# uguryagmur/RealTimeObjectDetection

Measured on AMD Instinct MI355X. Metric: frames/sec YOLOv3 608x608 bs=8 (Darknet.forward + write_results; 2 batches in flight, write_results_async on a second stream), higher is better.
Workload: dtype f16x2-split (3 MFMA products, f32 accumulate); 1 GPU; YOLOv3 cfg 608x608 batch=8 per GPU, split-f16 MFMA conv + fused head + GPU NMS (BASELINE configs[2]); precision=f16s3, tiles=autotune (this run), parallelism=frame-shard x1, in_flight_batches=2, detections_last_step=1699, candidates_last_step=1914, f16_range_overflow=False

## Files before the change

### include/rtod.h

```cpp
#ifndef RTOD_H
#define RTOD_H

#include <stddef.h>
#include <stdint.h>

#ifdef __cplusplus
extern "C" {
#endif

typedef enum rtod_status {
    RTOD_OK = 0,
    RTOD_E_ARG = -1,
    RTOD_E_HIP = -2,
    RTOD_E_CFG = -3,
    RTOD_E_STATE = -4,
    RTOD_E_SIZE = -5
} rtod_status;

typedef struct rtod_plan rtod_plan;

typedef struct rtod_plan_info {
    int32_t n_layers;
    int32_t n_launches;
    int32_t height, width, max_batch;
// ... 14 lines not shown
    int32_t fused_pointwise;
    int64_t flops_per_frame;
    int64_t bytes_per_frame;
    int64_t weight_bytes;
} rtod_launch_info;

int rtod_version(void);
int rtod_last_error(char* buf, size_t len);
int rtod_device_count(int* out);

int rtod_plan_create(const char* cfg_text, size_t len, int height, int width, int max_batch,
                     int device, rtod_plan** out);
int rtod_plan_create_rect(const char* cfg_text, size_t len, int height, int width, int max_batch,
                          int device, rtod_plan** out);
int rtod_plan_destroy(rtod_plan* plan);
int rtod_plan_get_info(const rtod_plan* plan, rtod_plan_info* out);
int rtod_plan_get_launch(const rtod_plan* plan, int index, rtod_launch_info* out);
int rtod_plan_describe(const rtod_plan* plan, char* buf, size_t len, size_t* needed);
int rtod_plan_pack_weights(const rtod_plan* plan, const float* w, size_t n_floats, float* out, size_t capacity_floats,
                           size_t* needed_floats);
const char* rtod_conv_variant_name(int variant);
int rtod_conv_kernel_name(int variant, int epilogue, char* buf, size_t len);
int rtod_plan_launch_kernel_name(const rtod_plan* plan, int index, char* buf, size_t len);
int rtod_plan_set_precision(rtod_plan* plan, int mode);
int rtod_plan_set_option(rtod_plan* plan, const char* name, int value);
int rtod_plan_set_overflow_flag(rtod_plan* plan, int32_t* flag_dev);

int rtod_plan_load_weights(rtod_plan* plan, const float* w, size_t n_floats);

int rtod_forward(rtod_plan* plan, const float* x_dev, int batch, float* out_dev, void* stream);
int rtod_plan_autotune(rtod_plan* plan, const float* x_dev, int batch, float* out_dev, void* stream);
int rtod_plan_get_tiles(const rtod_plan* plan, int batch, int* variants, int capacity);
int rtod_plan_set_tiles(rtod_plan* plan, int batch, const int* variants, int count);
int rtod_forward_timed(rtod_plan* plan, const float* x_dev, int batch, float* out_dev,
                       void* stream, float* launch_ms);
int rtod_plan_set_train_decode(rtod_plan* plan, int train);
int rtod_plan_finish_decode(rtod_plan* plan, float* pred_dev, int batch, void* stream);
int rtod_plan_set_keep_all_layers(rtod_plan* plan, int keep);
int rtod_plan_layer_shape(const rtod_plan* plan, int layer, int* c, int* h, int* w);
int rtod_plan_read_layer(rtod_plan* plan, int layer, int batch, float* out_dev_nchw, void* stream);
int rtod_plan_bn_batch_stats(rtod_plan* plan, int layer, double* mean_host, double* var_host, int channels, void* stream);
int rtod_plan_bn_update_running(rtod_plan* plan, int batch, float* const* running_mean_dev, float* const* running_var_dev, int n_bn,
                                double momentum, void* stream);

int rtod_predict_transform(const float* raw_dev, int batch, int attrs, int grid, int n_anchors,
                           const float* anchors_wh, int inp_dim, int train, float* out_dev,
// ... 46 lines not shown
```

### realtimeobjectdetection_amd/_ffi.py

```python
import ctypes as C
import os

_HERE = os.path.dirname(os.path.abspath(__file__))
LIB_PATH = os.path.join(_HERE, os.environ.get("RTOD_LIB", "librtod.so"))


class RtodError(RuntimeError):
    def __init__(self, code, msg):
        super().__init__(f"librtod error {code}: {msg}")
        self.code = code


class PlanInfo(C.Structure):
    _fields_ = [("n_layers", C.c_int32), ("n_launches", C.c_int32), ("height", C.c_int32),
                ("width", C.c_int32), ("max_batch", C.c_int32), ("total_rows", C.c_int32),
                ("attrs", C.c_int32), ("n_weight_floats", C.c_int64),
                ("conv_flops_per_frame", C.c_int64), ("arena_bytes", C.c_int64),
                ("packed_weight_bytes", C.c_int64)]


class LaunchInfo(C.Structure):
    _fields_ = [("layer", C.c_int32), ("kind", C.c_int32), ("variant", C.c_int32),
                ("ksize", C.c_int32), ("stride", C.c_int32), ("cin", C.c_int32), ("cout", C.c_int32),
                ("hout", C.c_int32), ("wout", C.c_int32), ("fused_residual", C.c_int32),
                ("fused_decode", C.c_int32), ("fused_pointwise", C.c_int32), ("flops_per_frame", C.c_int64),
                ("bytes_per_frame", C.c_int64), ("weight_bytes", C.c_int64)]


class YoloHead(C.Structure):
    _fields_ = [("grid_h", C.c_int), ("grid_w", C.c_int), ("stride", C.c_int), ("n_anchors", C.c_int), ("anchors", C.c_int * 16)]


SIGNATURES = {
    "rtod_version": (C.c_int, []),
    "rtod_last_error": (C.c_int, [C.c_char_p, C.c_size_t]),
    "rtod_device_count": (C.c_int, [C.POINTER(C.c_int)]),
    "rtod_plan_create": (C.c_int, [C.c_char_p, C.c_size_t, C.c_int, C.c_int, C.c_int, C.c_int, C.POINTER(C.c_void_p)]),
    "rtod_plan_create_rect": (C.c_int, [C.c_char_p, C.c_size_t, C.c_int, C.c_int, C.c_int, C.c_int, C.POINTER(C.c_void_p)]),
    "rtod_plan_destroy": (C.c_int, [C.c_void_p]),
    "rtod_plan_get_info": (C.c_int, [C.c_void_p, C.POINTER(PlanInfo)]),
    "rtod_plan_get_launch": (C.c_int, [C.c_void_p, C.c_int, C.POINTER(LaunchInfo)]),
    "rtod_plan_describe": (C.c_int, [C.c_void_p, C.c_char_p, C.c_size_t, C.POINTER(C.c_size_t)]),
    "rtod_plan_pack_weights": (C.c_int, [C.c_void_p, C.c_void_p, C.c_size_t, C.c_void_p, C.c_size_t, C.POINTER(C.c_size_t)]),
    "rtod_conv_variant_name": (C.c_char_p, [C.c_int]),
    "rtod_conv_kernel_name": (C.c_int, [C.c_int, C.c_int, C.c_char_p, C.c_size_t]),
    "rtod_plan_launch_kernel_name": (C.c_int, [C.c_void_p, C.c_int, C.c_char_p, C.c_size_t]),
    "rtod_plan_set_precision": (C.c_int, [C.c_void_p, C.c_int]),
    "rtod_plan_set_option": (C.c_int, [C.c_void_p, C.c_char_p, C.c_int]),
    "rtod_plan_set_overflow_flag": (C.c_int, [C.c_void_p, C.c_void_p]),
    "rtod_plan_autotune": (C.c_int, [C.c_void_p, C.c_void_p, C.c_int, C.c_void_p, C.c_void_p]),
    "rtod_plan_get_tiles": (C.c_int, [C.c_void_p, C.c_int, C.POINTER(C.c_int), C.c_int]),
    "rtod_plan_set_tiles": (C.c_int, [C.c_void_p, C.c_int, C.POINTER(C.c_int), C.c_int]),
    "rtod_plan_load_weights": (C.c_int, [C.c_void_p, C.c_void_p, C.c_size_t]),
    "rtod_forward": (C.c_int, [C.c_void_p, C.c_void_p, C.c_int, C.c_void_p, C.c_void_p]),
    "rtod_forward_timed": (C.c_int, [C.c_void_p, C.c_void_p, C.c_int, C.c_void_p, C.c_void_p, C.POINTER(C.c_float)]),
    "rtod_plan_set_train_decode": (C.c_int, [C.c_void_p, C.c_int]),
    "rtod_plan_finish_decode": (C.c_int, [C.c_void_p, C.c_void_p, C.c_int, C.c_void_p]),
    "rtod_plan_set_keep_all_layers": (C.c_int, [C.c_void_p, C.c_int]),
    "rtod_plan_layer_shape": (C.c_int, [C.c_void_p, C.c_int, C.POINTER(C.c_int), C.POINTER(C.c_int), C.POINTER(C.c_int)]),
    "rtod_plan_read_layer": (C.c_int, [C.c_void_p, C.c_int, C.c_int, C.c_void_p, C.c_void_p]),
    "rtod_plan_bn_batch_stats": (C.c_int, [C.c_void_p, C.c_int, C.c_void_p, C.c_void_p, C.c_int, C.c_void_p]),
    "rtod_plan_bn_update_running": (C.c_int, [C.c_void_p, C.c_int, C.c_void_p, C.c_void_p, C.c_int, C.c_double, C.c_void_p]),
    "rtod_predict_transform": (C.c_int, [C.c_void_p, C.c_int, C.c_int, C.c_int, C.c_int, C.POINTER(C.c_float), C.c_int, C.c_int, C.c_void_p, C.c_void_p]),
    "rtod_confidence_mask": (C.c_int, [C.c_void_p, C.c_int64, C.c_int, C.c_float, C.c_void_p, C.c_void_p]),
    "rtod_bbox_iou": (C.c_int, [C.c_void_p, C.c_void_p, C.c_int, C.c_int, C.c_void_p, C.c_void_p]),
    "rtod_prep_image": (C.c_int, [C.c_void_p, C.c_int, C.c_int, C.c_int, C.c_int, C.c_void_p, C.c_void_p]),
    "rtod_prep_frames": (C.c_int, [C.c_void_p, C.c_int, C.c_int, C.c_int, C.c_int, C.c_int, C.c_int, C.c_void_p, C.c_void_p]),
    "rtod_write_results_workspace": (C.c_int, [C.c_int, C.c_int, C.POINTER(C.c_size_t)]),
# ... 44 lines not shown
```

### realtimeobjectdetection_amd/csrc/capi.cpp

```cpp
#include <cstring>
#include <new>

#include "plan.h"

namespace rtod { const std::string& last_error_string(); }
using namespace rtod;

struct rtod_plan { Plan p; };

#define RTOD_GUARD_BEGIN try {
#define RTOD_GUARD_END                                                                   \
    } catch (const std::bad_alloc&) { set_error("out of host memory"); return RTOD_E_ARG; } \
      catch (const std::exception& e) { set_error("internal error: %s", e.what()); return RTOD_E_ARG; } \
      catch (...) { set_error("internal error"); return RTOD_E_ARG; }

extern "C" {

int rtod_version(void) { return 100; }

int rtod_last_error(char* buf, size_t len) {
    if (!buf || !len) return RTOD_E_ARG;
    const std::string& e = last_error_string();
    const size_t n = e.size() < len - 1 ? e.size() : len - 1;
    memcpy(buf, e.data(), n);
    buf[n] = 0;
    return RTOD_OK;
// ... 85 lines not shown
    if (int rc = plan->p.pack_weights(w, n_floats, packed)) return rc;
    if (!packed.empty()) memcpy(out, packed.data(), sizeof(float) * packed.size());
    return RTOD_OK;
    RTOD_GUARD_END
}

const char* rtod_conv_variant_name(int variant) {
    if (variant == 100 + STEM2_VARIANT) return "conv_stem2_f16s3<2 x 4x16, stem + 3x3 s2 + 1x1>";
    if (variant >= 100) { const TileRef t = family_of(variant - 100); return t ? t.fam->info(t.mode).name : ""; }
    if (variant < 0 || variant % 10 >= CV_COUNT || variant / 10 > 2) return "";
    static const char* const kSliced[2][CV_COUNT] = {
        {"conv_igemm_f32<128x128,w64x64,k-slices>", "conv_igemm_f32<128x64,w64x32,k-slices>", "conv_igemm_f32<64x64,w32x32,k-slices>", "conv_igemm_f32<128x32,w32x32,k-slices>"},
        {"conv_igemm_f32<128x128,w64x64,wg per k-slice>", "conv_igemm_f32<128x64,w64x32,wg per k-slice>", "conv_igemm_f32<64x64,w32x32,wg per k-slice>", "conv_igemm_f32<128x32,w32x32,wg per k-slice>"}};
    if (variant >= 10) return kSliced[variant / 10 - 1][variant % 10];
    return conv_variant_info(variant).name;
}

int rtod_conv_kernel_name(int variant, int epilogue, char* buf, size_t len) {
    if (!buf || len == 0) { set_error("conv_kernel_name: null buffer"); return RTOD_E_ARG; }
    int n = -1;
    if (variant >= 100) { const TileRef t = family_of(variant - 100); if (t) n = t.fam->kernel_name(t.mode, epilogue, buf, len); }
    else n = conv_f32_kernel_name(variant, buf, len);
    if (n < 0 || (size_t)n >= len) { set_error("conv_kernel_name: unknown variant %d or buffer too small", variant); return RTOD_E_ARG; }
    return RTOD_OK;
}

int rtod_plan_launch_kernel_name(const rtod_plan* plan, int index, char* buf, size_t len) {
    RTOD_GUARD_BEGIN
    if (!plan || !buf || len == 0 || index < 0 || index >= (int)plan->p.launches.size()) { set_error("launch_kernel_name: bad args"); return RTOD_E_ARG; }
    rtod_launch_info li;
    plan->p.fill_launch_info(index, &li, plan->p.tuned.empty() ? plan->p.max_batch : plan->p.tuned.rbegin()->first);
    buf[0] = 0;
    if (li.kind != LK_CONV || li.flops_per_frame == 0) return RTOD_OK;
    int epi = li.fused_decode ? 2 : (li.fused_pointwise ? (li.fused_residual ? 4 : 3) : (li.fused_residual ? 1 : 0));
    if (plan->p.precision == 2 && li.variant >= 100) epi |= EPI_F16;
    if (plan->p.raw_launch(plan->p.launches[index]) && li.variant >= 100) epi = EPI_RAW;
    int n = -1;
    if (li.variant == 100 + STEM2_VARIANT) n = conv_stem2_kernel_name(li.fused_pointwise, buf, len);
    else return rtod_conv_kernel_name(li.variant, epi, buf, len);
    if (n < 0 || (size_t)n >= len) { set_error("launch_kernel_name: buffer too small"); return RTOD_E_ARG; }
    return RTOD_OK;
    RTOD_GUARD_END
}

int rtod_plan_set_precision(rtod_plan* plan, int mode) {
    if (!plan || mode < 0 || mode > 2) { set_error("set_precision: mode must be 0 (fp32), 1 (f16 split) or 2 (plain f16)"); return RTOD_E_ARG; }
// ... 258 lines not shown
```

### realtimeobjectdetection_amd/csrc/plan.h

```cpp
#pragma once
#include <functional>
#include <map>
#include <string>
#include <vector>

#include "rtod_internal.h"

namespace rtod {

enum LayerType { LT_CONV = 0, LT_SHORTCUT, LT_ROUTE, LT_UPSAMPLE, LT_MAXPOOL, LT_YOLO };
const char* layer_type_name(int t);

struct Layer {
    int index = 0;
    int type = LT_CONV;
    int cin = 0, cout = 0, hin = 0, win = 0, hout = 0, wout = 0;
    int size = 0, stride = 1, pad = 0;
    bool bn = false;
    int act = 0;
    bool nearest = false;
    bool decode_v5 = false;
    int pool_pad = 0;
    std::vector<int> srcs;
    std::vector<std::pair<int, int>> anchors;
// ... 61 lines not shown
    double* d_bn_partial = nullptr;
    int64_t bn_partial_count = 0;
    float* d_bn_raw = nullptr;
    int64_t bn_raw_floats = 0;
    float* d_scratch = nullptr;
    int64_t scratch_floats = 0;
    bool weights_loaded = false;
    int train_decode = 0;
    int precision = 0;
    bool keep_all = false;
    bool opt_fuse_pointwise = true;
    bool opt_stem_kernel = true;
    bool opt_band_kernel = true;
    bool opt_bn_batch_stats = false;
    bool opt_bn_batch_split = false;
    bool opt_bn_split_narrow = false;
    bool opt_fuse_bn_pool = true;
    bool opt_k_slices = true;
    bool opt_k_slice_workgroups = true;
    bool opt_k_slices_split = false;
    bool opt_stem2_kernel = true;
    bool opt_patch_kernel = true;
    bool opt_ring_kernel = true;
    bool opt_pwd_kernel = true;
    bool opt_fuse_shortcut = true;
    bool opt_fuse_decode = true;
    bool opt_zero_copy_concat = true;
    bool opt_narrow_cin = false;
    bool opt_stem_pool = false;
    bool opt_fuse_stem_pool = true;
    int opt_force_f16s3_variant = -1;
    int opt_force_f32_variant = -1;
    int32_t* overflow_flag = nullptr;
    std::vector<hipEvent_t> events;

    ~Plan();
    int parse(const std::string& cfg_text);
    int resolve_shapes();
    int plan_buffers();
    DecodeArgs decode_args(const Layer& yolo) const;
    int replan_or(const std::function<void()>& restore);
    void assign_arena();
    void layout_weights();
    bool uses_split(const Layer& L) const;
    int check_split_supported(int mode) const;
    int pack_weights(const float* w, size_t n, std::vector<float>& packed) const;
// ... 45 lines not shown
```

### realtimeobjectdetection_amd/csrc/plan_build.cpp

```cpp
#include "plan.h"

#include <algorithm>
#include <cstdarg>
#include <sstream>

namespace rtod {

static thread_local std::string g_err;

void set_error(const char* fmt, ...) {
    char buf[1024];
    va_list ap;
    va_start(ap, fmt);
    vsnprintf(buf, sizeof(buf), fmt, ap);
    va_end(ap);
    g_err = buf;
}
const std::string& last_error_string() { return g_err; }

int hip_fail(hipError_t e, const char* what) {
    if (e == hipSuccess) return RTOD_OK;
    set_error("HIP error %d (%s) at %s", (int)e, hipGetErrorString(e), what);
    return RTOD_E_HIP;
}
// ... 14 lines not shown
}

static int resolve_alias(const std::vector<Layer>& layers, int i) {
    while (layers[i].alias_of >= 0) i = layers[i].alias_of;
    return i;
}

void Plan::reset_planning() {
    for (auto& L : layers) { L.fused_into = -1; L.fused_away = false; L.buf = -1; L.coff = 0; L.alias_of = -1; L.bn_pool = -1; }
    bufs.clear(); launches.clear(); convs.clear(); input_buf = -1;
    tuned.clear(); tune_cache.clear(); tuning.clear();
}

int Plan::set_option(const char* name, int value) {
    if (!name) { set_error("set_option: null name"); return RTOD_E_ARG; }
    if (d_weights) { set_error("set_option: must be called before rtod_plan_load_weights"); return RTOD_E_STATE; }
    static const struct { const char* name; bool Plan::*flag; } kFlags[] = {
        {"fuse_pointwise", &Plan::opt_fuse_pointwise}, {"ring_kernel", &Plan::opt_ring_kernel}, {"pwd_kernel", &Plan::opt_pwd_kernel},
        {"stem2_kernel", &Plan::opt_stem2_kernel}, {"k_slices", &Plan::opt_k_slices}, {"bn_batch_stats", &Plan::opt_bn_batch_stats},
        {"bn_batch_split", &Plan::opt_bn_batch_split}, {"bn_split_narrow", &Plan::opt_bn_split_narrow}, {"fuse_bn_pool", &Plan::opt_fuse_bn_pool},
        {"k_slice_workgroups", &Plan::opt_k_slice_workgroups}, {"k_slices_split", &Plan::opt_k_slices_split}, {"patch_kernel", &Plan::opt_patch_kernel},
        {"stem_kernel", &Plan::opt_stem_kernel}, {"band_kernel", &Plan::opt_band_kernel}, {"fuse_shortcut", &Plan::opt_fuse_shortcut},
        {"fuse_decode", &Plan::opt_fuse_decode}, {"zero_copy_concat", &Plan::opt_zero_copy_concat}, {"narrow_cin", &Plan::opt_narrow_cin},
        {"stem_pool", &Plan::opt_stem_pool}, {"fuse_stem_pool", &Plan::opt_fuse_stem_pool},
    };
    const std::string k(name);
    bool* flag = nullptr; int* num = nullptr;
    for (const auto& f : kFlags) if (k == f.name) flag = &(this->*f.flag);
    if (k == "force_f16s3_variant") num = &opt_force_f16s3_variant;
    else if (k == "force_f32_variant") num = &opt_force_f32_variant;
    else if (!flag) { set_error("set_option: unknown option '%s'", name); return RTOD_E_ARG; }
    if (flag == &opt_bn_batch_stats && value && height != width) { set_error("set_option: bn_batch_stats is not supported on a rectangular plan (%dx%d)", height, width); return RTOD_E_ARG; }
    const bool old_flag = flag ? *flag : false; const int old_num = num ? *num : 0;
    if (flag) *flag = value != 0; else *num = value;
    return replan_or([&] { if (flag) *flag = old_flag; else *num = old_num; });
}

int Plan::replan_or(const std::function<void()>& restore) {
    reset_planning();
    int rc = plan_buffers();
    if (!rc && precision >= 1) rc = check_split_supported(precision);
    if (rc) {
        const std::string msg = last_error_string();
        restore();
        reset_planning();
        (void)plan_buffers();
        set_error("%s", msg.c_str());
// ... 371 lines not shown
```

### realtimeobjectdetection_amd/csrc/plan_tiles.cpp

```cpp
#include "plan.h"

#include <algorithm>
#include <mutex>

namespace rtod {

int Plan::choose_variant(const Layer& L, int batch) const {
    if (opt_force_f32_variant >= 0 && opt_force_f32_variant < CV_COUNT) return opt_force_f32_variant;
    if (L.cout <= 32) return CV_128x32;
    if (L.cout <= 64) return CV_128x64;
    const int64_t M = (int64_t)batch * L.hout * L.wout;
    const int64_t big = ((M + 127) / 128) * ((L.cout + 127) / 128);
    return big >= 512 ? CV_128x128 : CV_64x64;
}

int Plan::f32_slice_mode(const Launch& l, int batch, int variant) const {
    const PackedConv& pc = convs[l.conv_slot];
    if (pc.split || pc.stem || pc.slice_chunks <= 0) return 0;
    const Layer& L = layers[l.layer];
    const ConvVariantInfo& vi = conv_variant_info(variant);
    const int64_t M = (int64_t)batch * L.hout * L.wout;
    const int64_t tiles = ((M + vi.bm - 1) / vi.bm) * ((L.cout + vi.bn - 1) / vi.bn);
    const int64_t S = (pc.Kpad / 32 + pc.slice_chunks - 1) / pc.slice_chunks;
    return (opt_k_slice_workgroups && d_scratch && tiles < 512 && S * M * pc.Npad <= scratch_floats) ? 2 : 1;
}

bool Plan::tile_legal(const Launch& l, int v) const {
    const TileRef t = family_of(v);
    if (!t || l.kind != LK_CONV || l.conv_slot < 0 || !convs[l.conv_slot].split) return false;
    const PackedConv& pc = convs[l.conv_slot];
    const Layer& L = layers[l.layer];
    if (precision == 2 && !t.f16()) return false;
    if (raw_launch(l) && !t.raw()) return false;
    if (pc.narrow || t.is(TF_C16)) return pc.narrow && t.is(TF_C16);
    if (pc.ks_chunks > 0 || t.is(TF_KS)) return pc.ks_chunks > 0 && t.is(TF_KS);
    if (pc.band) return t.is(TF_BAND) && conv_band_mode_valid(t.mode, L.cin, L.hin, L.win);
    const bool hosts_pw = l.pw_guest >= 0 && pw_active(), plain = l.out_layer != -2 && !hosts_pw, same_map = L.hout == L.hin && L.wout == L.win;
    switch (t.fam->id) {
        case TF_GENERIC: return !(hosts_pw && t.fam->info(t.mode).bn < L.cout);
        case TF_BAND: return t.bandd_wide() && opt_band_kernel && plain && same_map && pc.Npad % 128 == 0 && pc.K == pc.Kpad &&
                             conv_bandd_wide_supported(L.size, L.stride, L.pad, pc.cin_p, L.win);
        case TF_RING: return !hosts_pw && L.act <= 1;
        case TF_PWD: return opt_pwd_kernel && plain && same_map && conv_pwd_supported(L.size, L.stride, L.pad, pc.cin_p);
        case TF_PATCH: return plain && L.act <= 1 && L.hout == L.hin && conv_patch_supported(L.size, L.stride, L.pad, L.cin, L.cout) &&
                              conv_patch_mode_valid(t.mode, L.cin, L.cout);
    }
    return false;
}

int Plan::default_tile(const Launch& l, int batch) const {
    const PackedConv& pc = convs[l.conv_slot];
    const Layer& L = layers[l.layer];
    const int64_t M = (int64_t)batch * L.hout * L.wout;
    if (pc.narrow) return tile_id(TF_C16, conv_c16_default_mode(L.cout, M));
    if (pc.ks_chunks > 0) return tile_id(TF_KS, ((M + 63) / 64) * ((L.cout + 63) / 64) < 512 ? 1 : 0);
    if (pc.band) {
        if (precision != 2 && !raw_launch(l)) return tile_id(TF_BAND, conv_band_default_mode(L.cin, L.hin, L.win));
        const TileFamily& B = tile_family(TF_BAND);
        for (int m = 0; m < B.modes; ++m) if (tile_legal(l, B.base + m)) return B.base + m;
        return B.base + B.f16_from;
    }
    const int64_t gn = (L.cout + 127) / 128;
    const int g = L.cout <= 64 ? HV_128x64 : ((M + 127) / 128) * gn >= 512 ? HV_128x128 : ((M + 63) / 64) * gn >= 512 ? HV_64x128 : HV_64x64;
    return tile_legal(l, g) ? g : HV_128x128_8W;
}

int Plan::variant_for(const Launch& l, int batch) const {
    int want = opt_force_f16s3_variant;
    if (want < 0) {
        auto it = tuned.find(batch);
        const size_t idx = &l - &launches[0];
        if (it != tuned.end() && idx < it->second.size()) want = it->second[idx];
    }
    int v = want >= 0 && tile_legal(l, want) ? want : default_tile(l, batch);
    if (family_of(v).ks_sched_b() && !(opt_k_slice_workgroups && ks_sched_b_fits(l, batch))) --v;
    return v;
}

std::vector<int> Plan::tile_candidates(const Launch& l, int batch) const {
    static const int kOrder[TF_COUNT] = {TF_GENERIC, TF_PATCH, TF_BAND, TF_PWD, TF_RING, TF_C16, TF_KS};
    const int cout = layers[l.layer].cout;
    const bool ks_b = opt_k_slice_workgroups && ks_sched_b_fits(l, batch);
    std::vector<int> cand;
    for (int f : kOrder) {
        if ((f == TF_RING && !opt_ring_kernel) || (f == TF_PATCH && !opt_patch_kernel)) continue;
        const TileFamily& F = tile_family(f);
        for (int m = 0; m < F.modes; ++m) {
            const int bn = F.info(m).bn;
            const bool too_wide = f == TF_GENERIC || f == TF_RING ? bn > 64 && bn > 2 * ((cout + 63) / 64 * 64)
                                : f == TF_PATCH ? bn > 64 && bn > cout
                                : f == TF_PWD ? bn > 128 && bn > (cout + 127) / 128 * 128 : false;
            if (too_wide || (family_of(F.base + m).ks_sched_b() && !ks_b) || !tile_legal(l, F.base + m)) continue;
            cand.push_back(F.base + m);
        }
    }
    return cand;
}

int Plan::launch_split_variant(ConvArgs& a, const PackedConv& pc, int v, hipStream_t s) const {
    const TileRef t = family_of(v);
    if (!t) { set_error("variant %d is no split-f16 tile", v); return RTOD_E_STATE; }
    if (precision == 2 && !t.f16()) { set_error("variant %d has no plain-f16 instance", v); return RTOD_E_STATE; }
    if (a.raw_out && !t.raw()) { set_error("variant %d has no raw-sum instance", v); return RTOD_E_STATE; }
// ... 7 lines not shown
    }
    if (pc.band != t.is(TF_BAND) && !(t.bandd_wide() && !pc.band)) {
        set_error(pc.band ? "variant %d requested for a band layer" : "band variant %d requested for a layer without band weights", v);
        return RTOD_E_STATE;
    }
    if (t.is(TF_KS)) {
        a.slice_chunks = pc.ks_chunks;
        a.partial = nullptr; a.partial_floats = 0;
        if (t.ks_sched_b()) { a.partial = d_scratch; a.partial_floats = scratch_floats; }
    }
    return t.fam->launch(a, t.mode, s);
}

static std::mutex g_tune_mutex;
static std::map<std::vector<int>, int> g_tune_memo;

int Plan::tune_launch(size_t li, ConvArgs& a, int batch, hipStream_t s) {
    const Launch& l = launches[li];
    const Layer& L = layers[l.layer];
    const bool pw = a.pw_wh != nullptr;
    const std::vector<int> key = {L.cin, L.cout, L.size, L.stride, L.hout, L.wout, l.in2_layer >= 0, l.out_layer == -2, pw ? a.pw_cout : 0,
                                  convs[l.conv_slot].band ? 1 : 0, opt_ring_kernel ? 1 : 0, opt_patch_kernel ? 1 : 0, opt_pwd_kernel ? 1 : 0, L.act,
                                  precision, L.hin, L.win, L.pad, convs[l.conv_slot].ks_chunks, opt_k_slice_workgroups ? 1 : 0,
                                  a.raw_out ? 1 : 0};
    auto it = tune_cache.find(key);
    if (it != tune_cache.end()) { tuning[li] = it->second; return RTOD_OK; }
    std::vector<int> gkey = key; gkey.push_back(device); gkey.push_back(batch);
    {
        std::lock_guard<std::mutex> lock(g_tune_mutex);
        auto git = g_tune_memo.find(gkey);
        if (git != g_tune_memo.end()) { tuning[li] = git->second; tune_cache[key] = git->second; return RTOD_OK; }
    }
    hipEvent_t e0, e1;
    RTOD_HIP(hipEventCreate(&e0)); RTOD_HIP(hipEventCreate(&e1));
    const std::vector<int> cand = tile_candidates(l, batch);
    int best_v = variant_for(l, batch);
    int rc = RTOD_OK;
    auto time_variant = [&](int v, int reps, int per, float& out_ms) -> int {
        out_ms = 1e30f;
        for (int rep = 0; rep < reps; ++rep) {
            (void)hipEventRecord(e0, s);
            for (int r = 0; r < per; ++r) { const int q = launch_split_variant(a, convs[l.conv_slot], v, s); if (q) return q; }
            (void)hipEventRecord(e1, s);
            if (hipEventSynchronize(e1) != hipSuccess) return hip_fail(hipGetLastError(), "autotune sync");
            float ms = 0.f; (void)hipEventElapsedTime(&ms, e0, e1);
            out_ms = std::min(out_ms, ms / per);
        }
// ... 57 lines not shown
```

### realtimeobjectdetection_amd/csrc/rtod_internal.h

```cpp
#pragma once
#include <hip/hip_runtime.h>
#if defined(RTOD_STAMPS) && !defined(RTOD_DIAG)
#define RTOD_DIAG 1
#endif
#include <algorithm>
#include <atomic>
#include <cstdint>
#include <cstdio>
#include <string>
#include <vector>

#include "../../include/rtod.h"

namespace rtod {

void set_error(const char* fmt, ...);
int hip_fail(hipError_t e, const char* what);

#define RTOD_HIP(expr)                                              \
    do {                                                            \
        hipError_t _e = (expr);                                     \
        if (_e != hipSuccess) return ::rtod::hip_fail(_e, #expr);   \
    } while (0)

// ... 159 lines not shown
constexpr int PATCH_VARIANT_BASE = 110;
bool conv_patch_supported(int ksize, int stride, int pad, int cin, int cout);
const ConvVariantInfo& conv_patch_mode_info(int mode);
int conv_patch_kernel_name(int mode, int epi, char* buf, size_t len);
int launch_conv_patch_f16s3(const ConvArgs& a, int mode, hipStream_t s);

constexpr int C16_MODES = 4;
constexpr int C16_VARIANT_BASE = 140;
constexpr bool conv_c16_supported(int cin) { return cin == 16; }
const ConvVariantInfo& conv_c16_mode_info(int mode);
int conv_c16_default_mode(int cout, int64_t m);
int conv_c16_kernel_name(int mode, int epi, char* buf, size_t len);
int launch_conv_c16_f16s3(const ConvArgs& a, int mode, hipStream_t s);

constexpr int KS_TILES = 3;
constexpr int KS_MODES = 2 * KS_TILES;
constexpr int KS_VARIANT_BASE = 150;
constexpr int64_t KS_SCRATCH_FLOATS = 8ll << 20;
const ConvVariantInfo& conv_ks_mode_info(int mode);
int conv_ks_slices(const ConvArgs& a);
int conv_ks_kernel_name(int mode, int epi, char* buf, size_t len);
int launch_conv_ks_f16s3(const ConvArgs& a, int mode, hipStream_t s);

enum TileFamilyId { TF_GENERIC = 0, TF_BAND, TF_RING, TF_PWD, TF_PATCH, TF_C16, TF_KS, TF_COUNT };
struct TileFamily {
    int id, base, modes;
    int f16_from;
    int raw_from;
    const ConvVariantInfo& (*info)(int mode);
    int (*kernel_name)(int mode, int epi, char* buf, size_t len);
    int (*launch)(const ConvArgs& a, int mode, hipStream_t s);
};
struct TileRef {
    const TileFamily* fam; int mode;
    explicit operator bool() const { return fam != nullptr; }
    bool is(int family) const { return fam && fam->id == family; }
    bool f16() const { return fam && mode >= fam->f16_from; }
    bool raw() const { return fam && mode >= fam->raw_from; }
    bool ks_sched_b() const { return is(TF_KS) && (mode & 1); }
    bool bandd_wide() const { return is(TF_BAND) && mode == BANDD_WIDE_MODE; }
};
TileRef family_of(int v);
const TileFamily& tile_family(int family);
inline int tile_id(int family, int mode) { return tile_family(family).base + mode; }

int launch_conv_stem(const float* x_nchw, const float* w, const float* bias, const View& out, int B, int H, int W,
                     int Ho, int Wo, int stride, int Cout, int leaky, hipStream_t s);
// ... 52 lines not shown
```

### realtimeobjectdetection_amd/csrc/split_tiles.cpp

```cpp
#include "rtod_internal.h"

namespace rtod {

static const TileFamily kFamilies[TF_COUNT] = {
    {TF_GENERIC, 0, HV_COUNT, 0, 0, conv_f16s3_variant_info, conv_f16s3_kernel_name, launch_conv_f16s3},
    {TF_BAND, BAND_VARIANT_BASE, BAND_MODES, BAND_LDS_MODES, BAND_LDS_MODES, conv_band_mode_info, conv_band_kernel_name, launch_conv_band_f16s3},
    {TF_RING, RING_VARIANT_BASE, RING_MODES, RING_MODES, RING_MODES, conv_ring_mode_info, conv_ring_kernel_name, launch_conv_ring_f16s3},
    {TF_PWD, PWD_VARIANT_BASE, PWD_MODES, 0, 0, conv_pwd_mode_info, conv_pwd_kernel_name, launch_conv_pwd_f16s3},
    {TF_PATCH, PATCH_VARIANT_BASE, PATCH_MODES, PATCH_MODES, PATCH_MODES, conv_patch_mode_info, conv_patch_kernel_name, launch_conv_patch_f16s3},
    {TF_C16, C16_VARIANT_BASE, C16_MODES, 0, 0, conv_c16_mode_info, conv_c16_kernel_name, launch_conv_c16_f16s3},
    {TF_KS, KS_VARIANT_BASE, KS_MODES, 0, KS_MODES, conv_ks_mode_info, conv_ks_kernel_name, launch_conv_ks_f16s3},
};
static_assert(HV_COUNT <= BAND_VARIANT_BASE, "generic tile ids end where the band family's begin");
static_assert(BAND_VARIANT_BASE + BAND_MODES <= RING_VARIANT_BASE, "band tile ids end where the ring family's begin");
static_assert(RING_VARIANT_BASE + RING_MODES <= PWD_VARIANT_BASE, "ring tile ids end where the pwd family's begin");
static_assert(PWD_VARIANT_BASE + PWD_MODES <= PATCH_VARIANT_BASE, "pwd tile ids end where the patch family's begin");
static_assert(PATCH_VARIANT_BASE + PATCH_MODES <= STEM2_VARIANT && STEM2_VARIANT < C16_VARIANT_BASE, "the fused stem's reported id lies between the patch and narrow families");
static_assert(C16_VARIANT_BASE + C16_MODES <= KS_VARIANT_BASE, "narrow tile ids end where the K-sliced family's begin");

TileRef family_of(int v) {
    for (const TileFamily& f : kFamilies)
        if (v >= f.base && v < f.base + f.modes) return {&f, v - f.base};
    return {nullptr, 0};
}

const TileFamily& tile_family(int family) { return kFamilies[family]; }

}
```

Before: 2573 frames/s.

## Add dedicated stride-2 3x3 split-f16 conv kernel family to autotune candidates

Adds a new tile family for 3x3 stride-2 pad-1 convolutions. It uses LDS DMA from precomputed per-lane origins and tap masks, a 3/4-stage ring, and register-pipelined weight loads, and it is offered to the autotuner as a candidate. The aim is to cut the generic kernel's address and gather overhead on YOLOv3's downsampling layers. It adds five compiled variants, a host-side address-map debug API and a larger autotune search space. It only helps where the autotuner picks it.

```diff
diff --git a/include/rtod.h b/include/rtod.h
--- a/include/rtod.h
+++ b/include/rtod.h
@@ -60,6 +60,8 @@
 const char* rtod_conv_variant_name(int variant);
 int rtod_conv_kernel_name(int variant, int epilogue, char* buf, size_t len);
 int rtod_plan_launch_kernel_name(const rtod_plan* plan, int index, char* buf, size_t len);
+int rtod_stride_two_address_map(int batch, int hi, int wi, int cin, int64_t in_ldc, int in_coff, int bm_rows, int tile, uint32_t* src,
+                         int32_t* lane_map, int32_t* frag_map);
 int rtod_plan_set_precision(rtod_plan* plan, int mode);
 int rtod_plan_set_option(rtod_plan* plan, const char* name, int value);
 int rtod_plan_set_overflow_flag(rtod_plan* plan, int32_t* flag_dev);
diff --git a/realtimeobjectdetection_amd/_ffi.py b/realtimeobjectdetection_amd/_ffi.py
--- a/realtimeobjectdetection_amd/_ffi.py
+++ b/realtimeobjectdetection_amd/_ffi.py
@@ -44,6 +44,7 @@
     "rtod_plan_pack_weights": (C.c_int, [C.c_void_p, C.c_void_p, C.c_size_t, C.c_void_p, C.c_size_t, C.POINTER(C.c_size_t)]),
     "rtod_conv_variant_name": (C.c_char_p, [C.c_int]),
     "rtod_conv_kernel_name": (C.c_int, [C.c_int, C.c_int, C.c_char_p, C.c_size_t]),
+    "rtod_stride_two_address_map": (C.c_int, [C.c_int, C.c_int, C.c_int, C.c_int, C.c_int64, C.c_int, C.c_int, C.c_int, C.c_void_p, C.c_void_p, C.c_void_p]),
     "rtod_plan_launch_kernel_name": (C.c_int, [C.c_void_p, C.c_int, C.c_char_p, C.c_size_t]),
     "rtod_plan_set_precision": (C.c_int, [C.c_void_p, C.c_int]),
     "rtod_plan_set_option": (C.c_int, [C.c_void_p, C.c_char_p, C.c_int]),
diff --git a/realtimeobjectdetection_amd/csrc/capi.cpp b/realtimeobjectdetection_amd/csrc/capi.cpp
--- a/realtimeobjectdetection_amd/csrc/capi.cpp
+++ b/realtimeobjectdetection_amd/csrc/capi.cpp
@@ -2,6 +2,7 @@
 #include <new>
 
 #include "plan.h"
+#include "conv_s2d_map.h"
 
 namespace rtod { const std::string& last_error_string(); }
 using namespace rtod;
@@ -133,6 +134,33 @@
     if (variant >= 100) { const TileRef t = family_of(variant - 100); if (t) n = t.fam->kernel_name(t.mode, epilogue, buf, len); }
     else n = conv_f32_kernel_name(variant, buf, len);
     if (n < 0 || (size_t)n >= len) { set_error("conv_kernel_name: unknown variant %d or buffer too small", variant); return RTOD_E_ARG; }
+    return RTOD_OK;
+}
+
+int rtod_stride_two_address_map(int batch, int hi, int wi, int cin, int64_t in_ldc, int in_coff, int bm_rows, int tile, uint32_t* src, int32_t* lane_map, int32_t* frag_map) {
+    if (batch <= 0 || hi <= 0 || wi <= 0 || cin <= 0 || cin % 32 || in_ldc <= 0 || in_coff < 0 || bm_rows <= 0 || bm_rows % 16 || tile < 0 || !src || !lane_map || !frag_map) {
+        set_error("s2d_address_map: bad args"); return RTOD_E_ARG;
+    }
+    S2dGeom g;
+    g.Hi = hi; g.Wi = wi; g.Ho = (hi - 1) / 2 + 1; g.Wo = (wi - 1) / 2 + 1; g.M = batch * g.Ho * g.Wo;
+    g.PS = (unsigned)in_ldc * 4u; g.lo_plane = (unsigned)in_ldc * 2u; g.in_coff = in_coff;
+    const int nsteps = 9 * (cin / 32), nblk = bm_rows / 16;
+    for (int blk = 0; blk < nblk; ++blk)
+        for (int lane = 0; lane < 64; ++lane) {
+            const int e = blk * 64 + lane, row = s2d_lane_row(blk, lane), q = s2d_lane_chunk(lane);
+            lane_map[e * 4 + 0] = row; lane_map[e * 4 + 1] = q;
+            lane_map[e * 4 + 2] = s2d_lane_lds(blk, lane, 0); lane_map[e * 4 + 3] = s2d_lane_lds(blk, lane, 1);
+            const S2dLane L = s2d_lane(g, tile * bm_rows + row, q);
+            for (int s = 0; s <= nsteps; ++s) {
+                const int tap = s % 9, chunk = s / 9;
+                const unsigned vo = s2d_voffset(L, tap, s2d_tap_offset(g, tap), s < nsteps);
+                for (int lo = 0; lo < 2; ++lo)
+                    src[((size_t)e * (nsteps + 1) + s) * 2 + lo] = vo == S2D_OOB ? 0xFFFFFFFFu : vo + s2d_chunk_offset(chunk, lo, g);
+            }
+        }
+    for (int i = 0; i < nblk; ++i)
+        for (int lane = 0; lane < 64; ++lane)
+            for (int lo = 0; lo < 2; ++lo) frag_map[(i * 64 + lane) * 2 + lo] = s2d_frag_lds(i, lane & 15, lane >> 4, lo);
     return RTOD_OK;
 }
 
diff --git a/realtimeobjectdetection_amd/csrc/conv_s2d_f16s3.hip b/realtimeobjectdetection_amd/csrc/conv_s2d_f16s3.hip
--- /dev/null
+++ b/realtimeobjectdetection_amd/csrc/conv_s2d_f16s3.hip
@@ -0,0 +1,214 @@
+#include "conv_bandd_common.h"
+#include "conv_s2d_map.h"
+
+namespace rtod {
+
+static_assert(S2D_OOB == OOB, "one out-of-range voffset");
+
+template <int BM, int NST, int MINW, int EPI>
+__global__ __launch_bounds__(256, MINW)
+void conv_s2d_f16s3_kernel(const ConvArgs a, const int grid_m, const int grid_n) {
+    static_assert(epi_kind(EPI) == EPI_SPLIT && !epi_f16(EPI) && !epi_raw(EPI), "plain split-f16 layers only");
+    constexpr int BN = 128, NW = 4, NT = NW * 64, TM = BM / 16, TN = 2;
+    static_assert(BM % 16 == 0 && TM >= 2, "tile rows");
+    static_assert(NST == 3 || NST == 4, "ring depth");
+    constexpr int STAGE = BM * 128;
+    constexpr int NPP = (TM + NW - 1) / NW;
+    constexpr int P = 2 * NPP, LB = 4;
+    constexpr int WAIT_B = 2 * P + 2 * LB;
+    constexpr int WAIT_A = NST == 3 ? P + 2 * LB : 2 * P + 2 * LB;
+    static_assert(NPP >= 1 && NPP <= 2 && WAIT_B <= 63, "counted waits");
+    constexpr int DUMP = NST * STAGE;
+    constexpr int RG = BM * BN * 4 <= 32768 ? BM : (BM / 2) * BN * 4 <= 32768 ? BM / 2 : BM / 4;
+
+    extern __shared__ __attribute__((aligned(16))) unsigned char smem[];
+    const int nwg = grid_m * grid_n;
+    int bid = blockIdx.x;
+    if (!a.xcd_by_n) bid = xcd_remap(bid, nwg);
+    const int bm = bid / grid_n, bn = bid - bm * grid_n;
+    const int tid = (int)threadIdx.x;
+    const int wave = __builtin_amdgcn_readfirstlane(tid >> 6), lane = tid & 63;
+    const int lr = lane & 15, lh = lane >> 4;
+    const int M = a.B * a.Ho * a.Wo;
+    const int m0 = bm * BM;
+
+    const __amdgpu_buffer_rsrc_t rs_a = buffer_rsrc(a.in, a.in_bytes);
+    const __amdgpu_buffer_rsrc_t rs_wh = buffer_rsrc(a.w_hi, a.w_bytes);
+    const __amdgpu_buffer_rsrc_t rs_wl = buffer_rsrc(a.w_lo, a.w_bytes);
+    const unsigned lds0 = (unsigned)(size_t)smem;
+    const int nsteps = 9 * (a.Cin / 32);
+
+    S2dGeom g;
+    g.Hi = a.Hi; g.Wi = a.Wi; g.Ho = a.Ho; g.Wo = a.Wo; g.M = M;
+    g.PS = (unsigned)a.in_ldc * 4u; g.lo_plane = (unsigned)a.in_ldc * 2u; g.in_coff = a.in_coff;
+    S2dLane dl[NPP];
+#pragma unroll
+    for (int k = 0; k < NPP; ++k) {
+        const int blk = wave + k * NW;
+        dl[k] = s2d_lane(g, blk < TM ? m0 + s2d_lane_row(blk, lane) : M, s2d_lane_chunk(lane));
+    }
+    int da_step = 0, da_tap = 0, da_chunk = 0, da_stage = 0;
+    auto dma_panel = [&]() __attribute__((always_inline)) {
+        asm volatile("" : "+s"(da_step), "+s"(da_tap), "+s"(da_chunk), "+s"(da_stage));
+        const bool live = da_step < nsteps;
+        const unsigned tap_off = s2d_tap_offset(g, da_tap);
+        const unsigned soff_hi = s2d_chunk_offset(da_chunk, 0, g), soff_lo = s2d_chunk_offset(da_chunk, 1, g);
+        const unsigned base = lds0 + (unsigned)(da_stage * STAGE);
+#pragma unroll
+        for (int k = 0; k < NPP; ++k) {
+            const int blk = wave + k * NW;
+            const unsigned dst = blk < TM ? base + (unsigned)s2d_lane_lds(blk, 0, 0) : lds0 + (unsigned)DUMP;
+            lds_dma_pair<S2D_LO>(rs_a, s2d_voffset(dl[k], da_tap, tap_off, live), soff_hi, soff_lo, dst);
+        }
+        ++da_step;
+        if (++da_tap == 9) { da_tap = 0; ++da_chunk; }
+        if (++da_stage == NST) da_stage = 0;
+    };
+
+    const int wn = wave;
+    const int n0 = bn * BN + wn * 32;
+    const unsigned bvoff = n0 + lr < a.Npad ? (unsigned)((n0 + lr) * 32 + lh * 8) * 2u : OOB;
+    const unsigned wchunk = (unsigned)a.Npad * (HBK * 2);
+    u32x4 Bq[3][TN][2];
+    int lb_step = 0;
+    auto load_b = [&](u32x4 (&q)[TN][2]) __attribute__((always_inline)) {
+        const unsigned vo = lb_step < nsteps ? bvoff : OOB;
+        const unsigned koff = (unsigned)lb_step * wchunk;
+        q[0][0] = buffer_load_b128(rs_wh, vo, koff);
+        q[0][1] = buffer_load_b128(rs_wl, vo, koff);
+        q[1][0] = buffer_load_b128<1024>(rs_wh, vo, koff);
+        q[1][1] = buffer_load_b128<1024>(rs_wl, vo, koff);
+        ++lb_step;
+    };
+
+    f32x4 acc[TM][TN];
+#pragma unroll
+    for (int i = 0; i < TM; ++i)
+#pragma unroll
+        for (int j = 0; j < TN; ++j)
+#pragma unroll
+            for (int e = 0; e < 4; ++e) acc[i][j][e] = 0.f;
+
+    typedef const f16x8 __attribute__((address_space(3))) lds_f16x8;
+    int xq = (int)lds0 + s2d_frag_lds(0, lr, lh, 0);
+    constexpr int LA = 2;
+    f16x8 Ah[LA + 1], Al[LA + 1];
+    auto read_unit = [&](int i, int stoff, f16x8& h, f16x8& l) __attribute__((always_inline)) {
+        const int o = xq + stoff;
+        h = *reinterpret_cast<lds_f16x8*>((unsigned)(o + S2D_BLOCK * i));
+        l = *reinterpret_cast<lds_f16x8*>((unsigned)(o + S2D_BLOCK * i + S2D_LO));
+    };
+
+    dma_panel();
+    load_b(Bq[0]);
+    dma_panel();
+    load_b(Bq[1]);
+
+    __builtin_amdgcn_s_setprio(2);
+    int rd_stage = 0;
+    auto step_body = [&](auto par_c) __attribute__((always_inline)) {
+        constexpr int par = decltype(par_c)::value;
+        asm volatile("" : "+v"(xq));
+        if constexpr (NST == 4) dma_panel();
+        vmcnt<WAIT_A>();
+        __builtin_amdgcn_sched_barrier(0);
+        __builtin_amdgcn_s_barrier();
+        asm volatile("" ::: "memory");
+        if constexpr (NST == 3) dma_panel();
+        const int stoff = rd_stage * STAGE;
+        if (++rd_stage == NST) rd_stage = 0;
+        read_unit(0, stoff, Ah[0], Al[0]);
+        if constexpr (LA == 2) read_unit(1, stoff, Ah[1], Al[1]);
+        __builtin_amdgcn_sched_barrier(0);
+        load_b(Bq[(par + 2) % 3]);
+        vmcnt<WAIT_B>();
+        tie_bset<false>(Bq[par]);
+        __builtin_amdgcn_sched_barrier(0);
+#pragma unroll
+        for (int i = 0; i < TM; ++i) {
+            if (i + LA < TM) read_unit(i + LA, stoff, Ah[(i + LA) % (LA + 1)], Al[(i + LA) % (LA + 1)]);
+            const f16x8 ah = Ah[i % (LA + 1)], al = Al[i % (LA + 1)];
+#pragma unroll
+            for (int jn = 0; jn < TN; ++jn) {
+                const f16x8 bh = __builtin_bit_cast(f16x8, Bq[par][jn][0]);
+                const f16x8 bl = __builtin_bit_cast(f16x8, Bq[par][jn][1]);
+                acc[i][jn] = __builtin_amdgcn_mfma_f32_16x16x32_f16(al, bh, acc[i][jn], 0, 0, 0);
+                acc[i][jn] = __builtin_amdgcn_mfma_f32_16x16x32_f16(ah, bl, acc[i][jn], 0, 0, 0);
+                acc[i][jn] = __builtin_amdgcn_mfma_f32_16x16x32_f16(ah, bh, acc[i][jn], 0, 0, 0);
+            }
+            __builtin_amdgcn_sched_barrier(0);
+        }
+#pragma unroll
+        for (int i = 0; i < TM; ++i) tie(acc[i][0], acc[i][1]);
+        asm volatile("s_waitcnt lgkmcnt(0)" ::: "memory");
+    };
+#pragma unroll 1
+    for (int s = 0; s < nsteps; s += 3) {
+        step_body(std::integral_constant<int, 0>{});
+        step_body(std::integral_constant<int, 1>{});
+        step_body(std::integral_constant<int, 2>{});
+    }
+    vmcnt<0>();
+    tie_bset<false>(Bq[0]); tie_bset<false>(Bq[1]); tie_bset<false>(Bq[2]);
+    __builtin_amdgcn_sched_barrier(0);
+    __builtin_amdgcn_s_setprio(0);
+
+    bandd_epilogue<BM, BN, BM, 32, NT, RG, false, 1, false, false>(a, acc, smem, bm, bn, tid, 0, wn, lr, lh, M, 0);
+}
+
+template <int BM, int NST>
+constexpr int s2d_lds_bytes() {
+    constexpr int RG = BM * 128 * 4 <= 32768 ? BM : (BM / 2) * 128 * 4 <= 32768 ? BM / 2 : BM / 4;
+    constexpr int ring = NST * BM * 128 + ((BM / 16) % 4 ? S2D_BLOCK : 0), epi = RG * 128 * 4;
+    return ring > epi ? ring : epi;
+}
+
+template <int BM, int NST, int MINW>
+static int launch_s2d(const ConvArgs& a, hipStream_t s) {
+    constexpr int BN = 128;
+    const int M = a.B * a.Ho * a.Wo;
+    const int gm = (M + BM - 1) / BM, gn = (a.Cout + BN - 1) / BN;
+    ConvArgs ax = a;
+    ax.xcd_by_n = (gn % 8 == 0 && (int64_t)a.Cout * a.K > (int64_t)M * a.Cin) ? 1 : 0;
+    constexpr int lds = s2d_lds_bytes<BM, NST>();
+    static_assert(lds <= 64 * 1024, "dynamic LDS without the opt-in");
+    hipLaunchKernelGGL((conv_s2d_f16s3_kernel<BM, NST, MINW, EPI_SPLIT>), dim3(gm * gn), dim3(256), lds, s, ax, gm, gn);
+    return hip_fail(hipGetLastError(), "conv_s2d_f16s3 launch");
+}
+
+#define RTOD_S2D_TILES(X) \
+    X(0, 128, 3, 3) X(1, 96, 3, 3) X(2, 64, 3, 3) X(3, 96, 4, 3) X(4, 64, 4, 3)
+
+#define RTOD_X_INFO(idx, bm, nst, minw) {bm, 128, "conv_s2d_f16s3<" #bm "x128,r" #nst ">"},
+static const ConvVariantInfo kS2dModes[S2D_MODES] = { RTOD_S2D_TILES(RTOD_X_INFO) };
+#undef RTOD_X_INFO
+const ConvVariantInfo& conv_s2d_mode_info(int idx) { return kS2dModes[idx < 0 || idx >= S2D_MODES ? 0 : idx]; }
+
+bool conv_s2d_supported(int ksize, int stride, int pad, int cin) { return ksize == 3 && stride == 2 && pad == 1 && cin >= 32 && cin % 32 == 0; }
+
+int conv_s2d_kernel_name(int idx, int epi, char* buf, size_t len) {
+#define RTOD_X_NAME(i, bm, nst, minw) \
+    if (idx == i) return snprintf(buf, len, "void rtod::conv_s2d_f16s3_kernel<" #bm ", " #nst ", " #minw ", %d>(rtod::ConvArgs, int, int)", epi);
+    RTOD_S2D_TILES(RTOD_X_NAME)
+#undef RTOD_X_NAME
+    return -1;
+}
+
+int launch_conv_s2d_f16s3(const ConvArgs& a, int idx, hipStream_t s) {
+    if (int rc = check_split_conv_args(a, "launch_conv_s2d", false)) return rc;
+    if (!conv_s2d_supported(a.kh, a.stride, a.pad, a.Cin) || a.kw != 3 || a.Ho != (a.Hi - 1) / 2 + 1 || a.Wo != (a.Wi - 1) / 2 + 1) {
+        set_error("launch_conv_s2d: unsupported shape (k=%d s=%d pad=%d Cin=%d %dx%d -> %dx%d)", a.kh, a.stride, a.pad, a.Cin, a.Hi, a.Wi, a.Ho, a.Wo); return RTOD_E_ARG;
+    }
+    if (a.dec.enabled || a.pw_wh || a.res || a.raw_out || a.f16 || a.leaky > 1) { set_error("launch_conv_s2d: plain split-f16 layers only (linear / leaky, no shortcut, decode, hosted conv, raw sums or plain f16)"); return RTOD_E_ARG; }
+    if (a.in_ldc % 8 || a.in_coff % 8 || a.K != a.Kpad || a.K != 9 * a.Cin || a.Npad % 128) { set_error("launch_conv_s2d: bad view / K"); return RTOD_E_ARG; }
+    if (a.B <= 0 || a.Ho <= 0 || a.Wo <= 0 || a.Cout <= 0) { set_error("launch_conv_s2d: empty shape"); return RTOD_E_ARG; }
+    switch (idx) {
+#define RTOD_X_CASE(i, bm, nst, minw) case i: return launch_s2d<bm, nst, minw>(a, s);
+        RTOD_S2D_TILES(RTOD_X_CASE)
+#undef RTOD_X_CASE
+    }
+    set_error("launch_conv_s2d: mode %d unsupported", idx);
+    return RTOD_E_ARG;
+}
+
+}
diff --git a/realtimeobjectdetection_amd/csrc/conv_s2d_map.h b/realtimeobjectdetection_amd/csrc/conv_s2d_map.h
--- /dev/null
+++ b/realtimeobjectdetection_amd/csrc/conv_s2d_map.h
@@ -0,0 +1,44 @@
+#pragma once
+#include <hip/hip_runtime.h>
+#include <cstdint>
+
+namespace rtod {
+
+constexpr unsigned S2D_OOB = 0x80000000u;
+constexpr int S2D_BLOCK = 2048, S2D_LO = 1024;
+
+struct S2dGeom {
+    int Hi, Wi, Ho, Wo;
+    int M;
+    unsigned PS;
+    unsigned lo_plane;
+    int in_coff;
+};
+
+struct S2dLane { unsigned origin, taps; };
+
+__host__ __device__ constexpr int s2d_lane_row(int blk, int lane) { return blk * 16 + (lane >> 2); }
+__host__ __device__ constexpr int s2d_lane_chunk(int lane) { return (lane & 3) ^ ((lane >> 3) & 3); }
+__host__ __device__ constexpr int s2d_lane_lds(int blk, int lane, int lo) { return blk * S2D_BLOCK + lo * S2D_LO + lane * 16; }
+__host__ __device__ constexpr int s2d_frag_lds(int i, int lr, int lh, int lo) { return i * S2D_BLOCK + lo * S2D_LO + lr * 64 + ((lh ^ ((lr >> 1) & 3)) << 4); }
+
+__host__ __device__ __forceinline__ S2dLane s2d_lane(const S2dGeom& g, int m, int q) {
+    S2dLane L = {0u, 0u};
+    if (m >= g.M) return L;
+    const int hw = g.Ho * g.Wo;
+    const int b = m / hw, r = m - b * hw;
+    const int oy = r / g.Wo, ox = r - oy * g.Wo;
+    const int iy0 = 2 * oy - 1, ix0 = 2 * ox - 1;
+    L.origin = (unsigned)((b * g.Hi + iy0) * g.Wi + ix0) * g.PS + (unsigned)(g.in_coff + 8 * q) * 2u;
+#pragma unroll
+    for (int t = 0; t < 9; ++t)
+        if ((unsigned)(iy0 + t / 3) < (unsigned)g.Hi && (unsigned)(ix0 + t % 3) < (unsigned)g.Wi) L.taps |= 1u << t;
+    return L;
+}
+__host__ __device__ __forceinline__ unsigned s2d_tap_offset(const S2dGeom& g, int tap) { return (unsigned)((tap / 3) * g.Wi + tap % 3) * g.PS; }
+__host__ __device__ __forceinline__ unsigned s2d_chunk_offset(int chunk, int lo, const S2dGeom& g) { return (unsigned)chunk * 64u + (lo ? g.lo_plane : 0u); }
+__host__ __device__ __forceinline__ unsigned s2d_voffset(const S2dLane& L, int tap, unsigned tap_off, bool live) {
+    return (live && ((L.taps >> tap) & 1u)) ? L.origin + tap_off : S2D_OOB;
+}
+
+}
diff --git a/realtimeobjectdetection_amd/csrc/plan.h b/realtimeobjectdetection_amd/csrc/plan.h
--- a/realtimeobjectdetection_amd/csrc/plan.h
+++ b/realtimeobjectdetection_amd/csrc/plan.h
@@ -107,6 +107,7 @@
     bool opt_stem2_kernel = true;
     bool opt_patch_kernel = true;
     bool opt_ring_kernel = true;
+    bool opt_s2d_kernel = true;
     bool opt_pwd_kernel = true;
     bool opt_fuse_shortcut = true;
     bool opt_fuse_decode = true;
diff --git a/realtimeobjectdetection_amd/csrc/plan_build.cpp b/realtimeobjectdetection_amd/csrc/plan_build.cpp
--- a/realtimeobjectdetection_amd/csrc/plan_build.cpp
+++ b/realtimeobjectdetection_amd/csrc/plan_build.cpp
@@ -60,7 +60,7 @@
         {"k_slice_workgroups", &Plan::opt_k_slice_workgroups}, {"k_slices_split", &Plan::opt_k_slices_split}, {"patch_kernel", &Plan::opt_patch_kernel},
         {"stem_kernel", &Plan::opt_stem_kernel}, {"band_kernel", &Plan::opt_band_kernel}, {"fuse_shortcut", &Plan::opt_fuse_shortcut},
         {"fuse_decode", &Plan::opt_fuse_decode}, {"zero_copy_concat", &Plan::opt_zero_copy_concat}, {"narrow_cin", &Plan::opt_narrow_cin},
-        {"stem_pool", &Plan::opt_stem_pool}, {"fuse_stem_pool", &Plan::opt_fuse_stem_pool},
+        {"stem_pool", &Plan::opt_stem_pool}, {"fuse_stem_pool", &Plan::opt_fuse_stem_pool}, {"s2d_kernel", &Plan::opt_s2d_kernel},
     };
     const std::string k(name);
     bool* flag = nullptr; int* num = nullptr;
diff --git a/realtimeobjectdetection_amd/csrc/plan_tiles.cpp b/realtimeobjectdetection_amd/csrc/plan_tiles.cpp
--- a/realtimeobjectdetection_amd/csrc/plan_tiles.cpp
+++ b/realtimeobjectdetection_amd/csrc/plan_tiles.cpp
@@ -44,6 +44,8 @@
         case TF_PWD: return opt_pwd_kernel && plain && same_map && conv_pwd_supported(L.size, L.stride, L.pad, pc.cin_p);
         case TF_PATCH: return plain && L.act <= 1 && L.hout == L.hin && conv_patch_supported(L.size, L.stride, L.pad, L.cin, L.cout) &&
                               conv_patch_mode_valid(t.mode, L.cin, L.cout);
+        case TF_S2D: return opt_s2d_kernel && precision == 1 && plain && l.in2_layer < 0 && L.act <= 1 && L.size == 3 && L.stride == 2 && L.pad == 1 &&
+                            pc.cin_p % 32 == 0 && pc.Npad % 128 == 0 && pc.K == pc.Kpad && conv_s2d_supported(L.size, L.stride, L.pad, pc.cin_p);
     }
     return false;
 }
@@ -78,7 +80,7 @@
 }
 
 std::vector<int> Plan::tile_candidates(const Launch& l, int batch) const {
-    static const int kOrder[TF_COUNT] = {TF_GENERIC, TF_PATCH, TF_BAND, TF_PWD, TF_RING, TF_C16, TF_KS};
+    static const int kOrder[TF_COUNT] = {TF_GENERIC, TF_PATCH, TF_BAND, TF_PWD, TF_S2D, TF_RING, TF_C16, TF_KS};
     const int cout = layers[l.layer].cout;
     const bool ks_b = opt_k_slice_workgroups && ks_sched_b_fits(l, batch);
     std::vector<int> cand;
@@ -132,7 +134,7 @@
     const std::vector<int> key = {L.cin, L.cout, L.size, L.stride, L.hout, L.wout, l.in2_layer >= 0, l.out_layer == -2, pw ? a.pw_cout : 0,
                                   convs[l.conv_slot].band ? 1 : 0, opt_ring_kernel ? 1 : 0, opt_patch_kernel ? 1 : 0, opt_pwd_kernel ? 1 : 0, L.act,
                                   precision, L.hin, L.win, L.pad, convs[l.conv_slot].ks_chunks, opt_k_slice_workgroups ? 1 : 0,
-                                  a.raw_out ? 1 : 0};
+                                  a.raw_out ? 1 : 0, opt_s2d_kernel ? 1 : 0};
     auto it = tune_cache.find(key);
     if (it != tune_cache.end()) { tuning[li] = it->second; return RTOD_OK; }
     std::vector<int> gkey = key; gkey.push_back(device); gkey.push_back(batch);
diff --git a/realtimeobjectdetection_amd/csrc/rtod_internal.h b/realtimeobjectdetection_amd/csrc/rtod_internal.h
--- a/realtimeobjectdetection_amd/csrc/rtod_internal.h
+++ b/realtimeobjectdetection_amd/csrc/rtod_internal.h
@@ -205,7 +205,14 @@
 int conv_ks_kernel_name(int mode, int epi, char* buf, size_t len);
 int launch_conv_ks_f16s3(const ConvArgs& a, int mode, hipStream_t s);
 
-enum TileFamilyId { TF_GENERIC = 0, TF_BAND, TF_RING, TF_PWD, TF_PATCH, TF_C16, TF_KS, TF_COUNT };
+constexpr int S2D_MODES = 5;
+constexpr int S2D_VARIANT_BASE = 170;
+bool conv_s2d_supported(int ksize, int stride, int pad, int cin);
+const ConvVariantInfo& conv_s2d_mode_info(int mode);
+int conv_s2d_kernel_name(int mode, int epi, char* buf, size_t len);
+int launch_conv_s2d_f16s3(const ConvArgs& a, int mode, hipStream_t s);
+
+enum TileFamilyId { TF_GENERIC = 0, TF_BAND, TF_RING, TF_PWD, TF_PATCH, TF_C16, TF_KS, TF_S2D, TF_COUNT };
 struct TileFamily {
     int id, base, modes;
     int f16_from;
diff --git a/realtimeobjectdetection_amd/csrc/split_tiles.cpp b/realtimeobjectdetection_amd/csrc/split_tiles.cpp
--- a/realtimeobjectdetection_amd/csrc/split_tiles.cpp
+++ b/realtimeobjectdetection_amd/csrc/split_tiles.cpp
@@ -10,6 +10,7 @@
     {TF_PATCH, PATCH_VARIANT_BASE, PATCH_MODES, PATCH_MODES, PATCH_MODES, conv_patch_mode_info, conv_patch_kernel_name, launch_conv_patch_f16s3},
     {TF_C16, C16_VARIANT_BASE, C16_MODES, 0, 0, conv_c16_mode_info, conv_c16_kernel_name, launch_conv_c16_f16s3},
     {TF_KS, KS_VARIANT_BASE, KS_MODES, 0, KS_MODES, conv_ks_mode_info, conv_ks_kernel_name, launch_conv_ks_f16s3},
+    {TF_S2D, S2D_VARIANT_BASE, S2D_MODES, S2D_MODES, S2D_MODES, conv_s2d_mode_info, conv_s2d_kernel_name, launch_conv_s2d_f16s3},
 };
 static_assert(HV_COUNT <= BAND_VARIANT_BASE, "generic tile ids end where the band family's begin");
 static_assert(BAND_VARIANT_BASE + BAND_MODES <= RING_VARIANT_BASE, "band tile ids end where the ring family's begin");
@@ -17,6 +18,7 @@
 static_assert(PWD_VARIANT_BASE + PWD_MODES <= PATCH_VARIANT_BASE, "pwd tile ids end where the patch family's begin");
 static_assert(PATCH_VARIANT_BASE + PATCH_MODES <= STEM2_VARIANT && STEM2_VARIANT < C16_VARIANT_BASE, "the fused stem's reported id lies between the patch and narrow families");
 static_assert(C16_VARIANT_BASE + C16_MODES <= KS_VARIANT_BASE, "narrow tile ids end where the K-sliced family's begin");
+static_assert(KS_VARIANT_BASE + KS_MODES <= S2D_VARIANT_BASE && S2D_VARIANT_BASE >= 170, "ids 0 - 169 are pinned: the stride-2 family starts at 170");
 
 TileRef family_of(int v) {
     for (const TileFamily& f : kFamilies)
```

New measurement: 2603 frames/s (median of 2 runs). No clear change (+1.2%).
